# Triton-AI/Triton-Racer-Sim

Measured on AMD Instinct MI355X. Metric: env-steps/s (whole node) at N envs x 120x160 RGB, higher is better.
Workload: dtype f32 state / f64 nearest-point / u8 image; 1 GPU; 1024 envs/GPU x 1 GPU, bicycle physics + L1 nearest point + 120x160 RGB pinhole rasteriser = BASELINE configs[2], generated_track 1185 pts, synthetic controls seed 0x5EED, auto-reset; envs_total=1024, envs_per_gpu=1024, img_h=120, img_w=160, depth=False, steps_per_launch=1, step_mode=resident worker (posted steps), prewarm_steps=8400, launcher=self

## Files before the change

### triton-racer-sim_amd/csrc/trsim_env.hpp

```cpp
#pragma once
#include <hip/hip_runtime.h>

#include <algorithm>
#include <cstdint>
#include <cstring>
#include <string>

#include "../../include/trsim.h"
#include "trsim_device.hpp"
#include "trsim_mem.hpp"
#include "trsim_tables.hpp"

namespace trsim { struct Resident; struct Comm; }

struct trs_env {
    trs_config cfg{};
    int device = 0, n = 0, H = 0, W = 0, cu_count = 0;
    hipStream_t sP = nullptr;
    hipEvent_t ev[8] = {};
    trsim::DevBuf<> slab;
    trsim::DevBuf<uint8_t> img[2];
    bool uniform_ok[2] = {false, false};
    trsim::DevBuf<float> depth[2];
    trsim::DevBuf<> blob_p;
    trsim::DevBuf<> blob_r;
    trsim::DevBuf<float> tangent, start_yaw;
    trsim::DevBuf<float4> cam;
    trsim::DevBuf<float> cam_pitch;
    trsim::DevBuf<float> dpitch;
    bool hilly = false;
    trsim::HillBlock hill_host{};
    trs_camera camera{};
    bool lens_on = false;
    trsim::LensTables lens;
    trsim::DevBuf<> lens_dev;
    size_t lens_pal_off = 0;
    bool light_on = false;
    const float* light = nullptr;
    trsim::DevBuf<float> light_own;
    trsim::DevBuf<unsigned long long> stats;
    trsim::DevBuf<double> loc_q; trsim::DevBuf<int32_t> loc_out; int loc_cap = 0;
    trsim::DevBuf<uint8_t> pre;
    trs_pre_config frame_filter{}; bool has_frame_filter = false, filter_dynamic = false;
    trsim::PinnedBuf<> pinned;
    trsim::DevBuf<int32_t> mux_state; int mux_tick = 0;
    trsim::DevBuf<uint8_t> tmp_in, tmp_out; trsim::DevBuf<float> tmp_f; size_t tmp_cap = 0;
    trsim::DevBuf<int> hsv_tab;
    trsim::DevBuf<unsigned> dyn_tab;
    trsim::DevBuf<> edge_scratch;
    trsim::PParams pp{};
    trsim::RParams rp{};
    trsim::TrackTables tab;
    bool track_loaded = false;
    int lds_p = 0, lds_r = 0, pts_bytes = 0;
    uint64_t step_count = 0;
// ... 62 lines not shown
```

### triton-racer-sim_amd/csrc/trsim_hip.hip

```cpp
#include <hip/hip_runtime.h>

#include <algorithm>
#include <array>
#include <cmath>
#include <cstdint>
#include <cstdio>
#include <cstring>
#include <string>
#include <utility>
#include <vector>

#include "../../include/trsim.h"
#include "../../include/trsim_spec.h"
#include "trsim_device.hpp"
#include "trsim_env.hpp"
#include "trsim_internal.hpp"
#include "trsim_tables.hpp"


#define TRS_EXPORT extern "C" __attribute__((visibility("default")))

namespace {


// ... 204 lines not shown
            if (sidx < 0) cam = lcam_prev[j];
            else {
                while (__hip_atomic_load(&pprog[j], __ATOMIC_ACQUIRE, __HIP_MEMORY_SCOPE_WORKGROUP) < sidx + 1) __builtin_amdgcn_s_sleep(2);
                cam = lcam[sidx * sp.cam_stride + j];
            }
            raster_lens_frame(p, rth, lb, lcache, (unsigned)lds_off_hill, frame_desc<DEPTH>(p, img, dep, e), cam);
            continue;
        }
        if constexpr (DYN) {
            if ((e - e_begin) % kDynBatch != 0) continue;
            const int nbatch = (e_end - e_begin + kDynBatch - 1) / kDynBatch;
            const int it = (sidx - sp.r_first) * nbatch + (e - e_begin) / kDynBatch;
            float4 cams[kDynBatch];
#pragma unroll
            for (int bi = 0; bi < kDynBatch; ++bi) {
                const int eb = e + bi;
                cams[bi] = make_float4(0.f, 0.f, 0.f, 1.f);
                if (eb < e_end) {
                    const int j = eb - e_begin;
                    if (sidx < 0) cams[bi] = lcam_prev[j];
                    else {
                        while (__hip_atomic_load(&pprog[j], __ATOMIC_ACQUIRE, __HIP_MEMORY_SCOPE_WORKGROUP) < sidx + 1) __builtin_amdgcn_s_sleep(2);
                        cams[bi] = lcam[sidx * sp.cam_stride + j];
                    }
                }
            }
            (void)raster_dyn_batch<DEPTH, LIGHT>(p, sp.fp, rth, smem, cams, min(kDynBatch, e_end - e), img, dep, e, it, tid, lane, [](bool) { return false; },
                                                 LIGHT ? llight + (e - e_begin) * 8 : nullptr, lds_off_lpal);
            continue;
        }
        const FrameDesc fd = frame_desc<DEPTH>(p, img, dep, e);
        RasterThread rl = rth;
        if constexpr (LIGHT && !HILLS && !DYN) rl.pal_off = light_wave_palette(p, lds_off_lpal, llight + (e - e_begin) * 8, lfilt, wave, lane);
        if (!sp.skip_uniform) raster_uniform_rows<DEPTH>(p, rl, fd);
        float4 cam;
        const int j = e - e_begin;
        if (sidx < 0) {
            cam = lcam_prev[j];
        } else {
            while (__hip_atomic_load(&pprog[j], __ATOMIC_ACQUIRE, __HIP_MEMORY_SCOPE_WORKGROUP) < sidx + 1) __builtin_amdgcn_s_sleep(2);
            cam = lcam[sidx * sp.cam_stride + j];
        }
        raster_ground_rows<DEPTH>(p, rl, fd, cam);
    }
    }
    STAMP(5);
}

using StepKernel = void (*)(SParams);
template <Variant V> StepKernel step_kernel_of()
{
    if constexpr (variant_built(V)) return &trs_step_kernel<(V & kVDepth) != 0, (V & kVDyn) != 0, (V & kVHills) != 0, (V & kVLens) != 0, (V & kVLight) != 0>;
    else return nullptr;
}
template <Variant... V> std::array<StepKernel, kVariants> step_kernel_table(std::integer_sequence<Variant, V...>) { return {step_kernel_of<V>()...}; }
const std::array<StepKernel, kVariants> kStepKernels = step_kernel_table(std::make_integer_sequence<Variant, kVariants>{});

#undef STAMP_STATS
struct PreParams {
    const uint8_t* src; uint8_t* dst;
    const int* hsv_tab;
    int n_img, H, W, gpr, gpe, r0, r1;
    int dynamic, color, n_filters;
    float contrast, offset;
    double baseline;
    unsigned lo[4], hi[4];
    int dst_ch[4];
// ... 555 lines not shown
#define HIPCHK(call)                                                                              \
    do {                                                                                          \
        hipError_t _e = (call);                                                                   \
        if (_e != hipSuccess) return fail(TRS_ERR_DEVICE, std::string(#call) + ": " + hipGetErrorString(_e)); \
    } while (0)

inline size_t align_up(size_t v, size_t a) { return (v + a - 1) / a * a; }

}

namespace {

const uint8_t* latest_frame(const trs_env* e) { return e->cfg.render ? e->img[(e->step_count + 1) & 1].get() : nullptr; }
const float* latest_depth(const trs_env* e) { return (e->cfg.render && e->cfg.depth) ? e->depth[(e->step_count + 1) & 1].get() : nullptr; }

int grid_of(const trs_env* e) { return (e->n + e->pp.envs_per_wg - 1) / e->pp.envs_per_wg; }

trsim::LdsFit handle_fit(const trs_env* e, Variant v, int lds_step) { return trsim::lds_fit(lds_step, e->pp.envs_per_wg, e->H, e->W, v, trsim::resident_on(e)); }
int steps_that_fit(const trs_env* e, Variant v, int lds_step) { return trsim::steps_that_fit(lds_step, e->pp.envs_per_wg, e->H, e->W, v); }
Variant variant_now(const trs_env* e) { return trsim::variant_of(e) & (e->track_loaded ? ~0u : ~kVHills); }

int sync_all(trs_env* e)
{
    if (e->res) { int rc = trsim::resident_quiesce(e); if (rc) return rc; }
    HIPCHK(hipStreamSynchronize(e->sP));
    return trsim::check_fault(e);
}

int quiesce(trs_env* e) { return e->res ? trsim::resident_quiesce(e) : TRS_OK; }

bool resident_steps(const trs_env* e) { return trsim::resident_on(e); }

int launch_step(trs_env* e, const float* st, const float* th, const float* br, const uint8_t* rs, int synth,
                int n_phys, int r_first, int r_last, uint64_t step_base, bool keep_uniform = false)
{
    const Variant v = trsim::variant_of(e);
    const StepKernel kernel = kStepKernels[v];
    if (!kernel) return fail(TRS_ERR_STATE, "internal error: no step kernel is built for this combination of camera, track, frame filter and lighting");
    SParams sp;
    const bool dyn = (v & kVDyn) != 0;
    sp.ph = e->pp;
    sp.ph.ctl_steer = st; sp.ph.ctl_thr = th; sp.ph.ctl_brk = br; sp.ph.ctl_reset = rs; sp.ph.ctl_stride = e->seq_stride;
    sp.ph.synth = synth; sp.ph.n_steps = n_phys; sp.ph.write_cam = 1; sp.ph.step_off = (uint32_t)step_base;
    sp.ra = e->rp;
    sp.img0 = e->img[0].get(); sp.img1 = e->img[1].get();
    sp.dep0 = e->depth[0].get(); sp.dep1 = e->depth[1].get();
    sp.n_phys = n_phys; sp.r_first = r_first; sp.r_last = r_last;
    sp.step_base = (unsigned)step_base;
    sp.lds_off_phys = e->lds_off_phys;
    sp.cam_stride = e->pp.envs_per_wg;
    const StepLds lds = step_lds_layout(e->lds_step, sp.cam_stride, e->H, e->W, v, n_phys);
    sp.lds_off_cam = lds.cam; sp.lds_off_prog = lds.prog;
    sp.skip_uniform = 0;
    for (int r = r_first; r <= r_last; ++r) {
        const int b = (int)((step_base + (uint64_t)(int64_t)r) & 1u);
        if (keep_uniform && r_first == r_last && e->uniform_ok[b] && !dyn && !e->lens_on && !e->light_on) sp.skip_uniform = 1;
        else e->uniform_ok[b] = !dyn && !e->lens_on && !e->light_on;
    }
    sp.fp = trsim::fparams_of(e, lds.dyn);
    hipLaunchKernelGGL(kernel, dim3(grid_of(e)), dim3(kBlock), lds.total, e->sP, sp);
    HIPCHK(hipGetLastError());
    return TRS_OK;
}

int run_camera_steps(trs_env* e, const float* st, const float* th, const float* br, const uint8_t* rs, int synth, int n, int per_launch, bool keep_uniform = false)
{
    const uint64_t s0 = e->step_count;
    int rc = TRS_OK;
    if (n == 1) {
        rc = launch_step(e, st, th, br, rs, synth, 1, 0, 0, s0, keep_uniform);
    } else {
        const int kmax = std::max(1, std::min(per_launch, steps_that_fit(e, trsim::variant_of(e), e->lds_step)));
        for (int done = 0; done < n && !rc;) {
            const int k = std::min(kmax, n - done);
            const size_t co = (size_t)done * (size_t)e->seq_stride;
            rc = launch_step(e, st ? st + co : st, th ? th + co : th, br ? br + co : br, done == 0 ? rs : nullptr, synth, k, done == 0 ? 0 : -1, k - 2, s0 + done);
            done += k;
        }
        if (!rc) rc = launch_step(e, st, th, br, nullptr, synth, 0, -1, -1, s0 + n);
    }
    if (rc) return rc;
    e->step_count += (uint64_t)n;
    return TRS_OK;
}

int run_physics_steps(trs_env* e, const float* st, const float* th, const float* br, const uint8_t* rs, int synth, int n, int per_launch)
{
    for (int done = 0; done < n;) {
        const int now = std::min(per_launch, n - done);
        PParams p = e->pp;
        const size_t co = (size_t)done * (size_t)e->seq_stride;
        p.ctl_steer = st ? st + co : st; p.ctl_thr = th ? th + co : th; p.ctl_brk = br ? br + co : br; p.ctl_reset = done == 0 ? rs : nullptr;
        p.ctl_stride = e->seq_stride;
        p.synth = synth; p.n_steps = now; p.write_cam = 0; p.step_off = (uint32_t)e->step_count;
        hipLaunchKernelGGL(trs_physics_kernel, dim3((e->n + kPhysBlock / 64 - 1) / (kPhysBlock / 64)), dim3(kPhysBlock), e->lds_p, e->sP, p);
        HIPCHK(hipGetLastError());
        e->step_count += (uint64_t)now;
        done += now;
    }
    return TRS_OK;
}

}
// ... 28 lines not shown
{
    e->cfg = *cfg; e->device = device; e->n = cfg->n_envs; e->H = cfg->img_h; e->W = cfg->img_w;
    hipDeviceProp_t prop;
    HIPCHK(hipGetDeviceProperties(&prop, device));
    e->cu_count = prop.multiProcessorCount > 0 ? prop.multiProcessorCount : 256;
    HIPCHK(hipStreamCreateWithFlags(&e->sP, hipStreamNonBlocking));
    for (auto& ev : e->ev) HIPCHK(hipEventCreate(&ev));
    HIPCHK(hipEventCreateWithFlags(&e->ev_order, hipEventDisableTiming));

    const size_t n = (size_t)e->n, fa = align_up(n * 4, 256), ba = align_up(n, 256);
    const size_t slab_bytes = fa * (10 + 2 + 3) + ba * 3;
    HIPCHK(e->slab.alloc(slab_bytes));
    HIPCHK(hipMemsetAsync(e->slab.get(), 0, slab_bytes, e->sP));
    unsigned char* c = e->slab.get();
    auto takef = [&](float*& ptr) { ptr = reinterpret_cast<float*>(c); c += fa; };
    PParams& k = e->pp;
    takef(k.x); takef(k.y); takef(k.z); takef(k.yaw); takef(k.v); takef(k.speed); takef(k.cte);
    takef(k.ep_return); takef(k.last_return); takef(k.steer_filt);
    k.seg_idx = reinterpret_cast<int32_t*>(c); c += fa;
    k.ep_len = reinterpret_cast<int32_t*>(c); c += fa;
    takef(e->ctl_steer); takef(e->ctl_thr); takef(e->ctl_brk);
    k.done = c; c += ba; k.pending = c; c += ba; e->ctl_reset = c; c += ba;
    HIPCHK(e->stats.alloc(64 * sizeof(unsigned long long)));
    HIPCHK(hipMemsetAsync(e->stats.get(), 0, e->stats.bytes(), e->sP));
    HIPCHK(e->cam.alloc((size_t)kRing * n * sizeof(float4)));
    HIPCHK(hipMemsetAsync(e->cam.get(), 0, e->cam.bytes(), e->sP));
    HIPCHK(e->cam_pitch.alloc((size_t)kRing * n * sizeof(float)));
    HIPCHK(hipMemsetAsync(e->cam_pitch.get(), 0, e->cam_pitch.bytes(), e->sP));
    k.stats = e->stats.get(); k.cam = e->cam.get();
    RParams& r = e->rp;
    r.stats = e->stats.get();
    if (cfg->render) {
        e->img_bytes = n * (size_t)e->H * e->W * 3;
        for (int b = 0; b < 2; ++b) {
            HIPCHK(e->img[b].alloc(e->img_bytes));
            HIPCHK(hipMemsetAsync(e->img[b].get(), 0, e->img_bytes, e->sP));
            if (cfg->depth) {
                HIPCHK(e->depth[b].alloc(n * (size_t)e->H * e->W * 4));
                HIPCHK(hipMemsetAsync(e->depth[b].get(), 0, e->depth[b].bytes(), e->sP));
            }
        }
    }
    k.n_envs = e->n; k.env_id_base = cfg->env_id_base;
    k.envs_per_wg = (e->n + e->cu_count - 1) / e->cu_count;
    r.n_envs = e->n; r.envs_per_wg = k.envs_per_wg;
    r.H = e->H; r.W = e->W; r.gpr = e->W / 4; r.gpe = r.gpr * e->H; r.depth = (cfg->render && cfg->depth) ? 1 : 0;
    k.dt = cfg->dt; k.max_steer = cfg->max_steer; k.inv_wheelbase = cfg->inv_wheelbase; k.accel_max = cfg->accel_max;
    k.drag_lin = cfg->drag_lin; k.roll_res = cfg->roll_res; k.brake_max = cfg->brake_max; k.v_max = cfg->v_max;
    k.v_rev_max = cfg->v_rev_max; k.offtrack_cte = cfg->offtrack_cte; k.offtrack_penalty = cfg->offtrack_penalty;
    k.cam_fwd = cfg->cam_fwd; k.auto_reset = cfg->auto_reset; k.seed = cfg->seed;
    if (r.gpr > kBlock) return fail(TRS_ERR_LIMIT, "img_w too large: more 4-pixel groups per row than threads per workgroup");
    if (r.gpr > kRasterThreads) return fail(TRS_ERR_LIMIT, "img_w too large: more 4-pixel groups per row than raster threads");
    r.rows_per_pass = kRasterThreads / r.gpr;
    HIPCHK(e->fault.alloc(64, hipHostMallocMapped | hipHostMallocCoherent));
    *e->fault.get() = 0ull;
    k.fault = e->fault.get(); r.fault = e->fault.get();
    HIPCHK(hipStreamSynchronize(e->sP));
    return TRS_OK;
}


}

TRS_EXPORT int trs_create(const trs_config* cfg, int device, trs_env** out)
{
    if (!cfg || !out) return fail(TRS_ERR_ARG, "null argument");
// ... 534 lines not shown
    int o[3] = {t[0], t[1], t[2]};
    if (c.color_filter_enabled) {
        const int r = t[0], g = t[1], b = t[2];
        const int v = std::max(r, std::max(g, b)), vmin = std::min(r, std::min(g, b)), diff = v - vmin;
        const int sdiv = v ? (int)std::lrint((255 << 12) / (1.0 * v)) : 0;
        const int hdiv = diff ? (int)std::lrint((180 << 12) / (6.0 * diff)) : 0;
        const int sat = (diff * sdiv + (1 << 11)) >> 12;
        int h = (v == r) ? (g - b) : ((v == g) ? (b - r + 2 * diff) : (r - g + 4 * diff));
        h = (h * hdiv + (1 << 11)) >> 12;
        if (h < 0) h += 180;
        const int hh = std::min(h, 255), ss = std::min(sat, 255);
        for (int f = 0; f < c.n_filters; ++f) {
            const bool in = hh >= c.hsv_lo[f][0] && hh <= c.hsv_hi[f][0] && ss >= c.hsv_lo[f][1] && ss <= c.hsv_hi[f][1] &&
                            v >= c.hsv_lo[f][2] && v <= c.hsv_hi[f][2];
            o[c.dst_channel[f]] = in ? 255 : 0;
        }
    }
    return (uint32_t)o[0] | ((uint32_t)o[1] << 8) | ((uint32_t)o[2] << 16);
}

int leading_uniform_rows(const std::vector<uint32_t>& pal, int H)
{
    int u = 0;
    while (u < H && pal[4 * u] == pal[4 * u + 1] && pal[4 * u] == pal[4 * u + 2] && pal[4 * u] == pal[4 * u + 3]) ++u;
    return u;
}

int upload_palette(trs_env* e)
{
    if (!e->track_loaded || !e->cfg.render) return TRS_OK;
    std::vector<uint32_t> pal(e->tab.palette);
    if (e->has_frame_filter && !e->filter_dynamic && !e->light_on)
        for (auto& c : pal) c = filter_colour(e->frame_filter, c);
    e->rp.uni_rows = (e->hilly || e->lens_on) ? 0 : leading_uniform_rows(pal, e->H);
    e->uniform_ok[0] = e->uniform_ok[1] = false;
    { int rq = sync_all(e); if (rq) return rq; }
    HIPCHK(hipMemcpy(e->blob_r.get() + e->rp.off_pal, pal.data(), pal.size() * 4, hipMemcpyHostToDevice));
    if (e->lens_on && e->lens_dev.get()) {
        std::vector<uint32_t> lp(e->lens.palette);
        if (e->has_frame_filter && !e->filter_dynamic)
            for (auto& c : lp) c = filter_colour(e->frame_filter, c);
        HIPCHK(hipMemcpy(e->lens_dev.get() + e->lens_pal_off, lp.data(), lp.size() * 4, hipMemcpyHostToDevice));
    }
    if (e->hilly || e->light_on) {
        const bool flt = e->has_frame_filter && !e->filter_dynamic;
        trsim::HillBlock& hb = e->hill_host;
        std::vector<uint32_t> sky(e->tab.sky);
        hb.far_rgb = e->tab.far_rgb;
        hb.filt = flt ? 1 : 0;
        hb.light = e->light_on ? e->light : nullptr;
        if (flt) {
            const trs_pre_config& c = e->frame_filter;
            if (!e->light_on) {
                for (auto& v : sky) v = filter_colour(c, v);
                hb.far_rgb = filter_colour(c, hb.far_rgb);
            }
            { int rc = ensure_hsv_table(e); if (rc) return rc; }
            hb.f_color = c.color_filter_enabled; hb.f_nfilters = c.n_filters; hb.f_contrast = c.contrast_ratio; hb.f_offset = c.contrast_offset;
            for (int k = 0; k < 4; ++k) {
                hb.f_lo[k] = (unsigned)trsim::pack_hsv(c.hsv_lo[k]);
                hb.f_hi[k] = (unsigned)trsim::pack_hsv(c.hsv_hi[k]);
                hb.f_dst[k] = c.dst_channel[k];
            }
            hb.hsv_tab = e->hsv_tab.get();
        }
        if (e->hilly) HIPCHK(hipMemcpy(e->blob_r.get() + hb.off_sky, sky.data(), sky.size() * 4, hipMemcpyHostToDevice));
        HIPCHK(hipMemcpy(e->blob_r.get() + trsim::hill_block_offset(e->rp.blob_bytes), &hb, sizeof hb, hipMemcpyHostToDevice));
    }
    return TRS_OK;
// ... 533 lines not shown
    out[0] = e->d2h_bytes; out[1] = e->h2d_bytes; out[2] = e->step_count; out[3] = 0;
    return TRS_OK;
}

TRS_EXPORT const char* trs_last_error(void) { return g_err.c_str(); }

bool trs_internal_view(trs_env* e, TrsEnvView* v)
{
    if (!e || !v) return false;
    if (quiesce(e)) return false;
    v->device = e->device; v->n = e->n; v->H = e->H; v->W = e->W; v->render = e->cfg.render;
    v->stream = e->sP;
    v->latest_frame = e->step_count > 0 ? latest_frame(e) : nullptr;
    v->speed = e->pp.speed; v->seg_idx = e->pp.seg_idx; v->n_points = e->pp.np;
    v->ctl_steer = e->ctl_steer; v->ctl_thr = e->ctl_thr; v->ctl_brk = e->ctl_brk;
    v->step_count = e->step_count;
    v->stats = e->stats.get();
    return true;
}
void** trs_internal_pilot_slot(trs_env* e) { return e ? &e->pilot : nullptr; }
const trs_pilot_tuning* trs_internal_pilot_tuning(trs_env* e) { return e && e->has_pilot_tuning ? &e->pilot_tuning : nullptr; }
void trs_internal_set_pilot_tuning(trs_env* e, const trs_pilot_tuning* t)
{
    if (!e) return;
    e->has_pilot_tuning = t != nullptr;
    if (t) e->pilot_tuning = *t;
}
int trs_internal_fail(int code, const std::string& msg) { return fail(code, msg); }
void trs_internal_count(trs_env* e, uint64_t d2h, uint64_t h2d) { if (e) { e->d2h_bytes += d2h; e->h2d_bytes += h2d; } }
int trs_internal_step_launch(trs_env* e, const float* d_st, const float* d_th, const float* d_br)
{
    if (!e || !e->track_loaded) return fail(TRS_ERR_STATE, "no track loaded");
    { int rq = quiesce(e); if (rq) return rq; }
    const int rc = e->cfg.render ? run_camera_steps(e, d_st, d_th, d_br, nullptr, 0, 1, 1, true) : run_physics_steps(e, d_st, d_th, d_br, nullptr, 0, 1, 1);
    if (!rc) trsim::resident_note_launch(e);
    return rc;
}
int trs_internal_replay_launch(trs_env* e, const float* st, const float* th, const float* br, const uint8_t* rs, int synth, uint64_t step)
{
    if (e->cfg.render) return launch_step(e, st, th, br, rs, synth, 1, 0, 0, step);
    PParams p = e->pp;
    p.ctl_steer = st; p.ctl_thr = th; p.ctl_brk = br; p.ctl_reset = rs; p.ctl_stride = 0;
    p.synth = synth; p.n_steps = 1; p.write_cam = 0; p.step_off = (uint32_t)step;
    hipLaunchKernelGGL(trs_physics_kernel, dim3((e->n + kPhysBlock / 64 - 1) / (kPhysBlock / 64)), dim3(kPhysBlock), e->lds_p, e->sP, p);
    HIPCHK(hipGetLastError());
    return TRS_OK;
}
void trs_internal_note(const std::string& msg) { g_err = msg; }
int trsim::sync_handle(trs_env* e) { return sync_all(e); }
int trsim::quiesce_handle(trs_env* e) { return quiesce(e); }
int trsim::check_fault(trs_env* e)
{
    if (e->fault.get() && __atomic_load_n(e->fault.get(), __ATOMIC_ACQUIRE) != 0ull)
        return fail(TRS_ERR_DEVICE, "a step kernel found its dynamic LDS segment at a non-zero offset and refused to run: frames and state are stale");
    return TRS_OK;
}

#ifdef TRS_DEBUG_PROBES
__global__ __launch_bounds__(1024) void trs_debug_poison_kernel(unsigned pattern, int bytes, int spin)
{
    u4v* d = reinterpret_cast<u4v*>(smem);
    for (int i = threadIdx.x; i < bytes / 16; i += blockDim.x) d[i] = (u4v)(pattern);
    __syncthreads();
    const long long t0 = clock64();
    while (clock64() - t0 < spin) __builtin_amdgcn_s_sleep(8);
}

// ... 34 lines not shown
```

### triton-racer-sim_amd/csrc/trsim_plan.hpp

```cpp
#pragma once
#include <cstddef>
#include <string>
#include <vector>

#include "trsim_tables.hpp"

#ifndef TRS_RASTER_WAVES
#define TRS_RASTER_WAVES 8
#endif

namespace trsim {

constexpr int kRasterThreads = 64 * TRS_RASTER_WAVES;
constexpr int kPhysBlock = 256;
constexpr int kCamDepth = 4;
constexpr int kSlotWords = 20;
constexpr int kLensPalBytes = 513 * 16;
constexpr int kDynTabWords = 512 + 768 + 4 + 256;

using Variant = unsigned;
constexpr Variant kVDepth = 1, kVDyn = 2, kVHills = 4, kVLens = 8, kVLight = 16, kVariants = 32;
constexpr Variant variant_bits(bool depth, bool dyn, bool hills, bool lens, bool light)
{
    return (depth ? kVDepth : 0u) | (dyn ? kVDyn : 0u) | (hills ? kVHills : 0u) | (lens ? kVLens : 0u) | (light ? kVLight : 0u);
// ... 74 lines not shown
    return wlds_slot_off(epw) + (size_t)kCamDepth * epw * kSlotWords * 4 + (size_t)epw * 64;
}

struct WorkerLds { int ctl, dyn, hill, light, total; };
TRS_HD inline int worker_lds_light(int hill, int H, Variant v) { return (hill + tabs_lds_bytes(H, v) + 15) & ~15; }
TRS_HD inline WorkerLds worker_lds_layout(int lds_step, int epw, int H, int W, Variant v)
{
    WorkerLds L;
    L.ctl = (lds_step + 15) & ~15;
    int end = (int)(L.ctl + wlds_bytes(epw) + 16);
    L.dyn = (end + 15) & ~15;
    if (v & kVDyn) end = L.dyn + dyn_lds_bytes(H);
    L.hill = (end + 15) & ~15;
    if (v & (kVHills | kVLens)) end = L.hill + tabs_lds_bytes(H, v);
    L.light = worker_lds_light(L.hill, H, v);
    L.total = (v & kVLight) ? L.light + light_lds_extra(H, W, kCamDepth * epw, (v & kVHills) != 0, (v & kVDyn) != 0) : end;
    return L;
}

inline int steps_that_fit(int lds_step, int epw, int H, int W, Variant v)
{
    int n = 0;
    while (n < 16 && step_lds_layout(lds_step, epw, H, W, v, n + 1).total <= 160 * 1024) ++n;
    return n;
}
inline bool resident_fits(int lds_step, int epw, int H, int W, Variant v) { return worker_lds_layout(lds_step, epw, H, W, v).total <= 160 * 1024; }
enum class LdsFit { ok, no_launch, no_worker };
inline LdsFit lds_fit(int lds_step, int epw, int H, int W, Variant v, bool resident)
{
    if (steps_that_fit(lds_step, epw, H, W, v) < 1) return LdsFit::no_launch;
    return resident && !resident_fits(lds_step, epw, H, W, v) ? LdsFit::no_worker : LdsFit::ok;
}

struct TrackLayout {
    struct Phys { int off_py, off_pz, off_tan, tan_in_lds, off_gstart, off_gpts, blob_bytes, off_scratch, pts_bytes, lds_p; } p;
    struct Raster { int map_pitch_b, off_rowtab, off_pal, off_depth, off_sky, blob_bytes, lds_r; } r;
    int lds_off_phys, lds_step;
};
int track_layout(const TrackTables& T, int H, bool render, int envs_per_wg, TrackLayout& L, std::string& err);
void pack_track_images(const TrackTables& T, int H, const TrackLayout& L, std::vector<unsigned char>& phys, std::vector<unsigned char>& raster);

}
```

### triton-racer-sim_amd/csrc/trsim_resident.hip

```cpp
#include <hip/hip_runtime.h>

#include <algorithm>
#include <array>
#include <atomic>
#include <chrono>
#include <cstdint>
#include <cstdlib>
#include <cstddef>
#include <cstring>
#include <mutex>
#include <string>
#include <utility>

#include "../../include/trsim.h"
#include "../../include/trsim_spec.h"
#include "trsim_device.hpp"
#include "trsim_env.hpp"
#include "trsim_internal.hpp"

#define TRS_EXPORT extern "C" __attribute__((visibility("default")))

namespace trsim {

constexpr int kSlots = 8;
// ... 12 lines not shown

struct Mailbox {
    alignas(64) uint64_t close;
    uint64_t posted;
    alignas(64) uint64_t exited;
    uint64_t consumed;
    uint64_t error;
    uint64_t started;
    alignas(64) uint64_t done[kSlots];
    alignas(64) WEntry ring[kSlots];
};

struct DevCtl {
    alignas(64) unsigned long long word;
    alignas(64) WEntry ring[kSlots];
    alignas(64) unsigned arrive[kSlots][8][16];
    alignas(64) unsigned top[kSlots][16];
    alignas(64) unsigned checkin[16];
    alignas(64) unsigned decision[16];
};

struct WParams {
    PParams ph;
    RParams ra;
    uint8_t *img0, *img1;
    float *dep0, *dep1;
    Mailbox* mb;
    DevCtl* dc;
    unsigned long long start;
    unsigned long long idle_ticks, life_ticks, safety_ticks;
    unsigned long long checkin_ticks;
    int lds_off_phys, lds_off_ctl, n_blocks;
    int lds_off_hill;
    FParams fp;
};
#ifndef TRS_RESIDENT_DIAG
#define TRS_RESIDENT_DIAG 0
#endif
constexpr int kDiag = TRS_RESIDENT_DIAG;

constexpr unsigned kDefaultLifeUs = 50000;
#ifndef TRS_PHYS_PRIO_MAX_ENVS
#define TRS_PHYS_PRIO_MAX_ENVS 1
#endif
constexpr unsigned kRetryMs0 = 100;

struct Resident {
    bool enabled = false, running = false;
    bool broken = false;
    PinnedBuf<Mailbox> mb;
    DevBuf<DevCtl> dc;
    hipStream_t sC = nullptr;
    uint64_t base = 0;
    uint64_t seen_done = 0;
    bool launched = false;
    bool fell_back = false;
    bool dc_ready = false; uint64_t dc_ready_for = 0;
    std::chrono::steady_clock::time_point t_launch{};
    std::chrono::steady_clock::time_point t_fallback{};
    unsigned retry_ms = kRetryMs0;
    unsigned idle_us = 2000;
    unsigned life_us = kDefaultLifeUs;
    PinnedBuf<> hctl;
    size_t hctl_slot = 0;
    int lds_bytes = 0, lds_off_ctl = 0, lds_off_dyn = 0, lds_off_hill = 0;
    long long pw_capacity_envs = 0;
    int pw_capacity_lds = -1;
};

}

namespace {

using namespace trsim;
using u64 = unsigned long long;

constexpr u64 kExitBit = 1ull << 63, kAbortBit = 1ull << 62, kCountMask = kAbortBit - 1;
constexpr u64 kExitNormal = 1ull, kExitNotCoresident = 2ull;
constexpr u64 kCloseLeave = 1ull, kCloseCancel = 2ull;
constexpr int kFellBack = trsim::kResidentFellBack;

constexpr int kMaxDevices = 64;
struct DeviceSlot { std::recursive_mutex mu; trs_env* owner = nullptr; };
DeviceSlot g_dev[kMaxDevices];
struct DevLock {
    std::unique_lock<std::recursive_mutex> lk;
    explicit DevLock(const trs_env* e) : lk(g_dev[(unsigned)e->device % kMaxDevices].mu) {}
};
inline DeviceSlot& slot_of(const trs_env* e) { return g_dev[(unsigned)e->device % kMaxDevices]; }
// ... 384 lines not shown
        }
        if (D.forwarder) {
            u64 t0 = 0;
            for (unsigned spins = 0; D.fwd < s; ++spins) {
                forward_arrivals(wp, l, D.fwd, lane);
                if (lds_load64(l.word) & kAbortBit) break;
                __builtin_amdgcn_s_sleep(2);
                if ((spins & 1023u) == 1023u) {
                    const u64 now = (u64)wall_clock64();
                    if (t0 == 0) t0 = now;
                    else if (now - t0 > wp.safety_ticks) { worker_abort(wp, l, 4u); break; }
                }
            }
        }
        return;
    }

    const RasterThread rth = raster_thread(p, smem, tid);
    trsim::LensBlock lb{};
    LensCacheWorker<DEPTH> lcache;
    if constexpr (LENS) {
        lb = *reinterpret_cast<const trsim::LensBlock*>(p.blob + trsim::lens_block_offset(p.blob_bytes));
        lens_cache_load(p, rth, lb, lcache);
    }
    int nu = 0, ng = 0;
    for (int v = rth.vstart; v < p.uni_rows; v += p.rows_per_pass) ++nu;
    for (int v = rth.vground; v < p.H; v += p.rows_per_pass) ++ng;
#pragma unroll
    for (int off = 32; off >= 1; off >>= 1) { nu = max(nu, __shfl_xor(nu, off, 64)); ng = max(ng, __shfl_xor(ng, off, 64)); }
    nu *= DEPTH ? 2 : 1; ng *= DEPTH ? 2 : 1;
    int own = 0;
    for (int j = wave; j < n_loc; j += kRasterThreads / 64) ++own;
    const int nuni = nu * n_loc, nstep = (nu + ng) * n_loc + 2 * own;
    const int lag = (2 * nstep + nuni <= 63) ? 3 : 2;
    unsigned char* optr = nullptr;
    {
        unsigned char* const tab[14] = {(unsigned char*)P.x, (unsigned char*)P.y, (unsigned char*)P.z, (unsigned char*)P.yaw, (unsigned char*)P.v,
                                        (unsigned char*)P.speed, (unsigned char*)P.cte, (unsigned char*)P.seg_idx, (unsigned char*)P.ep_return,
                                        (unsigned char*)P.ep_len, (unsigned char*)P.steer_filt, (unsigned char*)P.last_return,
                                        (unsigned char*)P.done, (unsigned char*)P.pending};
#pragma unroll
        for (int k = 0; k < 14; ++k) optr = lane == k ? tab[k] : optr;
    }
    Duties none{false, false, 0};
    u64 owed = wp.start;
    const bool probe = (kDiag & 4) && blockIdx.x == 7 && wave == 0;
    auto now_clk = [&]() -> u64 { u64 t; asm volatile("s_memtime %0\n\ts_waitcnt lgkmcnt(0)" : "=s"(t) :: "memory"); return t; };
    u64 t_post = 0, t_pose = 0, t_vm = 0, t_all = 0, t_mark = probe ? now_clk() : 0;
    for (u64 s = wp.start;; ++s) {
        const int r = (int)(s - wp.start);
        if (owed < s && (lds_load64(l.word) & kCountMask) <= s) {
            drain_vmem();
            for (; owed < s; ++owed) raster_arrive(l, owed, lane);
        }
        const u64 tp0 = probe ? now_clk() : 0;
        if (!wait_posted(wp, l, none, s, lane)) {
            drain_vmem();
            for (; owed < s; ++owed) raster_arrive(l, owed, lane);
            if (probe && lane == 0) {
                t_all = now_clk() - t_mark;
                atomicAdd(&p.stats[40], t_post); atomicAdd(&p.stats[41], t_pose); atomicAdd(&p.stats[42], t_vm); atomicAdd(&p.stats[43], t_all);
                atomicAdd(&p.stats[44], (u64)r);
            }
            return;
        }
        if (probe) t_post += now_clk() - tp0;
        uint8_t* const img = (s & 1ull) ? wp.img1 : wp.img0;
// ... 90 lines not shown
                    else if (lane < 14) __hip_atomic_store((__attribute__((address_space(1))) unsigned char*)(uintptr_t)optr + e, (unsigned char)(lane == 12 ? tel : 0u), __ATOMIC_RELAXED, __HIP_MEMORY_SCOPE_SYSTEM);
                }
            }
            continue;
        }
        if constexpr (LIGHT && !HILLS && !DYN) {
            for (int j = 0; j < n_loc; ++j) {
                const FrameDesc fd = frame_desc<DEPTH>(p, img, dep, e_begin + j);
                if (!wait_lds_ge(wp, l, nullptr, &l.pprog[j], r + 1, 3u, lane)) return;
                const float* const sl = l.slot + ((size_t)(r & (kCamDepth - 1)) * epw + j) * kSlotWords;
                const float4 cam = *reinterpret_cast<const float4*>(sl);
                const bool mine = (j % (kRasterThreads / 64)) == wave;
                unsigned tel = 0;
                if (mine) tel = __float_as_uint(sl[4 + min(lane, 12)]);
                RasterThread rl = rth;
                rl.pal_off = light_wave_palette(p, lds_off_lpal, lring + ((size_t)(r & (kCamDepth - 1)) * epw + j) * 8, lfilt, wave, lane);
                asm volatile("s_waitcnt lgkmcnt(0)" :: "v"(cam.x), "v"(cam.y), "v"(cam.z), "v"(cam.w), "v"(tel) : "memory");
                if (lane == 0) __hip_atomic_fetch_add(&l.rread[j], 1, __ATOMIC_RELAXED, __HIP_MEMORY_SCOPE_WORKGROUP);
                raster_uniform_rows<DEPTH>(p, rl, fd);
                if (j == 0)
                    while (s - owed >= keep) {
                        wait_vmcnt_le((int)(s - owed - 1) * nstep + nu);
                        raster_arrive(l, owed++, lane);
                    }
                raster_ground_rows<DEPTH>(p, rl, fd, cam);
                if (mine && !(kDiag & 2)) {
                    const size_t e = (size_t)(e_begin + j);
                    if (lane < 12) __hip_atomic_store((__attribute__((address_space(1))) unsigned*)(uintptr_t)optr + e, tel, __ATOMIC_RELAXED, __HIP_MEMORY_SCOPE_SYSTEM);
                    else if (lane < 14) __hip_atomic_store((__attribute__((address_space(1))) unsigned char*)(uintptr_t)optr + e, (unsigned char)(lane == 12 ? tel : 0u), __ATOMIC_RELAXED, __HIP_MEMORY_SCOPE_SYSTEM);
                }
            }
            continue;
        }
        const bool sweep = ahead == 0;
        if (sweep)
            for (int j = 0; j < n_loc; ++j) raster_uniform_rows<DEPTH>(p, rth, frame_desc<DEPTH>(p, img, dep, e_begin + j));
        for (int j = 0; j < n_loc; ++j) {
            const FrameDesc fd = frame_desc<DEPTH>(p, img, dep, e_begin + j);
            if (!sweep) raster_uniform_rows<DEPTH>(p, rth, fd);
            if (j == 0)
                while (s - owed >= keep) {
                    const u64 tv0 = probe ? now_clk() : 0;
                    if (!(kDiag & 1)) wait_vmcnt_le((int)(s - owed - 1) * nstep + (sweep ? nuni : nu));
                    if (probe) t_vm += now_clk() - tv0;
                    raster_arrive(l, owed++, lane);
                }
            const u64 tq0 = probe ? now_clk() : 0;
            if (!wait_lds_ge(wp, l, nullptr, &l.pprog[j], r + 1, 3u, lane)) return;
            if (probe) t_pose += now_clk() - tq0;
            const float* const sl = l.slot + ((size_t)(r & (kCamDepth - 1)) * epw + j) * kSlotWords;
            const float4 cam = *reinterpret_cast<const float4*>(sl);
            const bool mine = (j % (kRasterThreads / 64)) == wave;
            unsigned tel = 0;
            if (mine) tel = __float_as_uint(sl[4 + min(lane, 12)]);
            asm volatile("s_waitcnt lgkmcnt(0)" :: "v"(cam.x), "v"(cam.y), "v"(cam.z), "v"(cam.w), "v"(tel) : "memory");
            if (lane == 0) __hip_atomic_fetch_add(&l.rread[j], 1, __ATOMIC_RELAXED, __HIP_MEMORY_SCOPE_WORKGROUP);
            if constexpr (LENS) raster_lens_frame(p, rth, lb, lcache, (unsigned)wp.lds_off_hill, fd, cam);
            else raster_ground_rows<DEPTH>(p, rth, fd, cam);
            if (mine && !(kDiag & 2)) {
                const size_t e = (size_t)(e_begin + j);
                if (lane < 12) __hip_atomic_store((__attribute__((address_space(1))) unsigned*)(uintptr_t)optr + e, tel, __ATOMIC_RELAXED, __HIP_MEMORY_SCOPE_SYSTEM);
                else if (lane < 14) __hip_atomic_store((__attribute__((address_space(1))) unsigned char*)(uintptr_t)optr + e, (unsigned char)(lane == 12 ? tel : 0u), __ATOMIC_RELAXED, __HIP_MEMORY_SCOPE_SYSTEM);
            }
        }
    }
}

using WorkerKernel = void (*)(WParams);
template <Variant V> WorkerKernel worker_kernel_of()
{
    if constexpr (variant_built(V)) return &trs_worker_kernel<(V & kVDepth) != 0, (V & kVDyn) != 0, (V & kVHills) != 0, (V & kVLens) != 0, (V & kVLight) != 0>;
    else return nullptr;
}
template <Variant... V> std::array<WorkerKernel, kVariants> worker_kernel_table(std::integer_sequence<Variant, V...>) { return {worker_kernel_of<V>()...}; }
const std::array<WorkerKernel, kVariants> kWorkerKernels = worker_kernel_table(std::make_integer_sequence<Variant, kVariants>{});

// ... 181 lines not shown
    }
    const WorkerLds L = worker_lds_layout(e->lds_step, e->pp.envs_per_wg, e->H, e->W, variant_of(e));
    R->lds_off_ctl = L.ctl; R->lds_off_dyn = L.dyn; R->lds_off_hill = L.hill; R->lds_bytes = L.total;
    if (R->lds_bytes > 160 * 1024)
        return trs_internal_fail(TRS_ERR_LIMIT, e->hilly ? "the resident worker's LDS state and the per-env row tables of a track with elevation do not fit beside this track's tables: use TRS_STEP_LAUNCH"
                                                : e->lens_on ? "the resident worker's LDS state and the lens camera's palette do not fit beside this track's tables: use TRS_STEP_LAUNCH"
                                                : e->light_on ? "the resident worker's LDS state and the lit palettes of scene lighting do not fit beside this track's tables: use TRS_STEP_LAUNCH"
                                                            : "too many envs per workgroup for the resident worker's LDS state");
    return TRS_OK;
}

int evict(trs_env* other);

int worker_launch(trs_env* e, uint64_t start)
{
    Resident* R = e->res;
    Mailbox* mb = R->mb.get();
    { int rc = worker_fits(e); if (rc) return rc; }
    const WorkerKernel kernel = e->cfg.render ? kWorkerKernels[variant_of(e)] : nullptr;
    if (e->cfg.render && !kernel)
        return trs_internal_fail(TRS_ERR_STATE, "internal error: no resident worker is built for this combination of camera, track, frame filter and lighting");
    {
        DeviceSlot& D = slot_of(e);
        trs_env* const other = D.owner;
        if (other && other != e && other->res && other->res->running) (void)evict(other);
        D.owner = e;
    }
    host_store(&mb->exited, 0); host_store(&mb->consumed, start); host_store(&mb->error, 0);
    host_store(&mb->close, 0); host_store(&mb->started, 0);
    WParams wp{};
    wp.ph = e->pp; wp.ph.synth = 0; wp.ph.write_cam = 0; wp.ph.n_steps = 0; wp.ph.step_off = 0; wp.ph.ctl_stride = 0;
    wp.ra = e->rp;
    wp.img0 = e->img[0].get(); wp.img1 = e->img[1].get(); wp.dep0 = e->depth[0].get(); wp.dep1 = e->depth[1].get();
    e->uniform_ok[0] = e->uniform_ok[1] = false;
    wp.mb = mb; wp.dc = R->dc.get();
    wp.start = start;
    wp.idle_ticks = (unsigned long long)R->idle_us * 100ull;
    wp.life_ticks = (unsigned long long)R->life_us * 100ull;
    wp.safety_ticks = 200000000ull;
    wp.checkin_ticks = 200000ull;
    wp.lds_off_phys = e->lds_off_phys; wp.lds_off_ctl = R->lds_off_ctl; wp.lds_off_hill = R->lds_off_hill;
    const int grid = e->cfg.render ? (e->n + e->pp.envs_per_wg - 1) / e->pp.envs_per_wg : (e->n + kPwEnvs - 1) / kPwEnvs;
    wp.n_blocks = grid;
    if (!(R->dc_ready && R->dc_ready_for == start)) hipLaunchKernelGGL(trs_worker_init_kernel, dim3(1), dim3(256), 0, e->sP, R->dc.get(), (u64)start);
    R->dc_ready = false;
    if (e->cfg.render) {
        wp.fp = fparams_of(e, R->lds_off_dyn);
        hipLaunchKernelGGL(kernel, dim3(grid), dim3(kBlock), R->lds_bytes, e->sP, wp);
    } else {
        hipLaunchKernelGGL(trs_physics_worker_kernel, dim3(grid), dim3(kPwBlock), R->lds_bytes, e->sP, wp);
    }
    RCHK(hipGetLastError());
    R->running = true;
    R->t_launch = std::chrono::steady_clock::now();
    return TRS_OK;
}

int worker_error(trs_env* e)
{
    const uint64_t err = host_load(&e->res->mb->error);
    if (!err) return TRS_OK;
    e->res->broken = true;
    static const char* const what[] = {"", "waiting for a post", "camera ring back-pressure", "waiting for the physics team", "forwarding the last arrivals",
                                       "team barrier of the dynamic-brightness batch", "", "abort injected by trs_resident_debug_abort (test hook)", "",
                                       "dynamic LDS segment not at offset 0"};
    const unsigned code = (unsigned)(err >> 32);
    return trs_internal_fail(TRS_ERR_DEVICE, std::string("resident worker gave up (") + (code < 10 ? what[code] : "?") + ") in workgroup " +
                                                 std::to_string((unsigned)err));
}

int fall_back_to_launches(trs_env* e, uint64_t consumed, const char* why)
{
    Resident* R = e->res;
    const uint64_t posted = host_load(&R->mb->posted);
    R->enabled = false;
    R->fell_back = true;
    R->t_fallback = std::chrono::steady_clock::now();
    if (consumed > R->seen_done) R->seen_done = consumed;
    for (uint64_t s = consumed; s < posted; ++s) {
        const WEntry& en = R->mb->ring[s & (kSlots - 1)];
        if (en.seq != s + 1 || en.seq_lo != s + 1)
            return trs_internal_fail(TRS_ERR_DEVICE, "resident worker: the post of step " + std::to_string(s) + " is no longer in the ring");
        int rc = trs_internal_replay_launch(e, en.steer, en.thr, en.brk, en.reset, (int)en.synth, s);
        if (rc) return rc;
    }
    R->launched = true;
    R->base = R->seen_done = e->step_count;
    for (int k = 0; k < kSlots; ++k) { host_store(&R->mb->ring[k].seq, 0); host_store(&R->mb->ring[k].seq_lo, 0); host_store(&R->mb->done[k], 0); }
    trs_internal_note(std::string("resident worker: ") + why + " - another process's worker holds CUs of this GPU; the handle has gone back to TRS_STEP_LAUNCH "
                      "(resident mode is tried again by itself after " + std::to_string(R->retry_ms) + " ms; trs_get_step_mode tells)");
    return kFellBack;
}

int handle_exit(trs_env* e, bool relaunch = true)
{
    Resident* R = e->res;
    RCHK(hipStreamSynchronize(e->sP));
    R->running = false;
    int rc = worker_error(e);
    if (rc) return rc;
    const uint64_t consumed = host_load(&R->mb->consumed), posted = host_load(&R->mb->posted);
    if (host_load(&R->mb->exited) == kExitNotCoresident)
        return fall_back_to_launches(e, consumed, "the launch did not get every CU within 2 ms");
    if (consumed > R->seen_done) R->seen_done = consumed;
    if (host_load(&R->mb->started)) R->retry_ms = kRetryMs0;
    if (consumed < posted && relaunch) return worker_launch(e, consumed);
    if (consumed == posted) {
        hipLaunchKernelGGL(trs_worker_init_kernel, dim3(1), dim3(256), 0, e->sP, R->dc.get(), (u64)consumed);
        if (hipGetLastError() == hipSuccess) { R->dc_ready = true; R->dc_ready_for = consumed; }
    }
    return TRS_OK;
}

int evict(trs_env* other)
{
    Resident* R = other->res;
    int rc = TRS_OK;
    if (R->running) {
        host_store(&R->mb->close, kCloseLeave);
        rc = handle_exit(other, false);
    }
    return rc < 0 ? rc : TRS_OK;
}

int give_up_on_launch(trs_env* e)
{
    Resident* R = e->res;
    host_store(&R->mb->close, kCloseCancel);
    RCHK(hipStreamSynchronize(e->sP));
    R->running = false;
    int rc = worker_error(e);
    if (rc) return rc;
    return fall_back_to_launches(e, host_load(&R->mb->consumed), "the launch had not started after 250 ms");
}

int wait_done(trs_env* e, uint64_t s)
{
    Resident* R = e->res;
    if (s < R->seen_done) return TRS_OK;
    Mailbox* mb = R->mb.get();
    const auto t0 = std::chrono::steady_clock::now();
    auto fell_back = [&]() -> int {
        RCHK(hipStreamSynchronize(e->sP));
        R->launched = false;
        R->base = R->seen_done = e->step_count;
        return TRS_OK;
    };
    for (unsigned spins = 0;; ++spins) {
        if (host_load(&mb->done[s & (kSlots - 1)]) >= s + 1) { R->seen_done = s + 1; return TRS_OK; }
        if ((spins & 63u) == 63u) {
            if (R->running && host_load(&mb->exited)) {
                int rc = handle_exit(e);
                if (rc == kFellBack) return fell_back();
                if (rc) return rc;
                if (s < R->seen_done) return TRS_OK;
            } else if (!R->running) {
                if (host_load(&mb->posted) > R->seen_done) { int rc = worker_launch(e, R->seen_done); if (rc) return rc; }
            } else if ((spins & 4095u) == 4095u && !host_load(&mb->started) &&
                       std::chrono::steady_clock::now() - R->t_launch > std::chrono::milliseconds(250)) {
                int rc = give_up_on_launch(e);
                if (rc == kFellBack) return fell_back();
                if (rc) return rc;
            }
            if (host_load(&mb->error)) { (void)handle_exit(e); return worker_error(e); }
            if (std::chrono::steady_clock::now() - t0 > std::chrono::seconds(10))
// ... 258 lines not shown
```

Measured before the change: 108.3 million env-steps/s.

## Skip redundant uniform-row rasterisation in resident worker after double-buffered frames are primed

```diff
diff --git a/triton-racer-sim_amd/csrc/trsim_env.hpp b/triton-racer-sim_amd/csrc/trsim_env.hpp
--- a/triton-racer-sim_amd/csrc/trsim_env.hpp
+++ b/triton-racer-sim_amd/csrc/trsim_env.hpp
@@ -20,7 +20,7 @@
     hipEvent_t ev[8] = {};
     trsim::DevBuf<> slab;
     trsim::DevBuf<uint8_t> img[2];
-    bool uniform_ok[2] = {false, false};
+    trsim::UniformRows uniform_ok;
     trsim::DevBuf<float> depth[2];
     trsim::DevBuf<> blob_p;
     trsim::DevBuf<> blob_r;
diff --git a/triton-racer-sim_amd/csrc/trsim_hip.hip b/triton-racer-sim_amd/csrc/trsim_hip.hip
--- a/triton-racer-sim_amd/csrc/trsim_hip.hip
+++ b/triton-racer-sim_amd/csrc/trsim_hip.hip
@@ -260,7 +260,7 @@
         const FrameDesc fd = frame_desc<DEPTH>(p, img, dep, e);
         RasterThread rl = rth;
         if constexpr (LIGHT && !HILLS && !DYN) rl.pal_off = light_wave_palette(p, lds_off_lpal, llight + (e - e_begin) * 8, lfilt, wave, lane);
-        if (!sp.skip_uniform) raster_uniform_rows<DEPTH>(p, rl, fd);
+        if (!((sp.skip_uniform >> (abs_step & 1u)) & 1)) raster_uniform_rows<DEPTH>(p, rl, fd);
         float4 cam;
         const int j = e - e_begin;
         if (sidx < 0) {
@@ -882,13 +882,12 @@
 bool resident_steps(const trs_env* e) { return trsim::resident_on(e); }
 
 int launch_step(trs_env* e, const float* st, const float* th, const float* br, const uint8_t* rs, int synth,
-                int n_phys, int r_first, int r_last, uint64_t step_base, bool keep_uniform = false)
+                int n_phys, int r_first, int r_last, uint64_t step_base)
 {
     const Variant v = trsim::variant_of(e);
     const StepKernel kernel = kStepKernels[v];
     if (!kernel) return fail(TRS_ERR_STATE, "internal error: no step kernel is built for this combination of camera, track, frame filter and lighting");
     SParams sp;
-    const bool dyn = (v & kVDyn) != 0;
     sp.ph = e->pp;
     sp.ph.ctl_steer = st; sp.ph.ctl_thr = th; sp.ph.ctl_brk = br; sp.ph.ctl_reset = rs; sp.ph.ctl_stride = e->seq_stride;
     sp.ph.synth = synth; sp.ph.n_steps = n_phys; sp.ph.write_cam = 1; sp.ph.step_off = (uint32_t)step_base;
@@ -901,24 +900,20 @@
     sp.cam_stride = e->pp.envs_per_wg;
     const StepLds lds = step_lds_layout(e->lds_step, sp.cam_stride, e->H, e->W, v, n_phys);
     sp.lds_off_cam = lds.cam; sp.lds_off_prog = lds.prog;
-    sp.skip_uniform = 0;
-    for (int r = r_first; r <= r_last; ++r) {
-        const int b = (int)((step_base + (uint64_t)(int64_t)r) & 1u);
-        if (keep_uniform && r_first == r_last && e->uniform_ok[b] && !dyn && !e->lens_on && !e->light_on) sp.skip_uniform = 1;
-        else e->uniform_ok[b] = !dyn && !e->lens_on && !e->light_on;
-    }
+    sp.skip_uniform = (int)e->uniform_ok.skip_mask(v);
+    if (r_first <= r_last) e->uniform_ok.rendered(v, step_base + (uint64_t)(int64_t)r_first, (uint64_t)(r_last - r_first + 1));
     sp.fp = trsim::fparams_of(e, lds.dyn);
     hipLaunchKernelGGL(kernel, dim3(grid_of(e)), dim3(kBlock), lds.total, e->sP, sp);
     HIPCHK(hipGetLastError());
     return TRS_OK;
 }
 
-int run_camera_steps(trs_env* e, const float* st, const float* th, const float* br, const uint8_t* rs, int synth, int n, int per_launch, bool keep_uniform = false)
+int run_camera_steps(trs_env* e, const float* st, const float* th, const float* br, const uint8_t* rs, int synth, int n, int per_launch)
 {
     const uint64_t s0 = e->step_count;
     int rc = TRS_OK;
     if (n == 1) {
-        rc = launch_step(e, st, th, br, rs, synth, 1, 0, 0, s0, keep_uniform);
+        rc = launch_step(e, st, th, br, rs, synth, 1, 0, 0, s0);
     } else {
         const int kmax = std::max(1, std::min(per_launch, steps_that_fit(e, trsim::variant_of(e), e->lds_step)));
         for (int done = 0; done < n && !rc;) {
@@ -1013,6 +1008,7 @@
     r.stats = e->stats.get();
     if (cfg->render) {
         e->img_bytes = n * (size_t)e->H * e->W * 3;
+        e->uniform_ok.invalidate();
         for (int b = 0; b < 2; ++b) {
             HIPCHK(e->img[b].alloc(e->img_bytes));
             HIPCHK(hipMemsetAsync(e->img[b].get(), 0, e->img_bytes, e->sP));
@@ -1613,9 +1609,9 @@
     std::vector<uint32_t> pal(e->tab.palette);
     if (e->has_frame_filter && !e->filter_dynamic && !e->light_on)
         for (auto& c : pal) c = filter_colour(e->frame_filter, c);
+    { int rq = sync_all(e); if (rq) return rq; }
     e->rp.uni_rows = (e->hilly || e->lens_on) ? 0 : leading_uniform_rows(pal, e->H);
-    e->uniform_ok[0] = e->uniform_ok[1] = false;
-    { int rq = sync_all(e); if (rq) return rq; }
+    e->uniform_ok.invalidate();
     HIPCHK(hipMemcpy(e->blob_r.get() + e->rp.off_pal, pal.data(), pal.size() * 4, hipMemcpyHostToDevice));
     if (e->lens_on && e->lens_dev.get()) {
         std::vector<uint32_t> lp(e->lens.palette);
@@ -2215,7 +2211,7 @@
 {
     if (!e || !e->track_loaded) return fail(TRS_ERR_STATE, "no track loaded");
     { int rq = quiesce(e); if (rq) return rq; }
-    const int rc = e->cfg.render ? run_camera_steps(e, d_st, d_th, d_br, nullptr, 0, 1, 1, true) : run_physics_steps(e, d_st, d_th, d_br, nullptr, 0, 1, 1);
+    const int rc = e->cfg.render ? run_camera_steps(e, d_st, d_th, d_br, nullptr, 0, 1, 1) : run_physics_steps(e, d_st, d_th, d_br, nullptr, 0, 1, 1);
     if (!rc) trsim::resident_note_launch(e);
     return rc;
 }
diff --git a/triton-racer-sim_amd/csrc/trsim_plan.hpp b/triton-racer-sim_amd/csrc/trsim_plan.hpp
--- a/triton-racer-sim_amd/csrc/trsim_plan.hpp
+++ b/triton-racer-sim_amd/csrc/trsim_plan.hpp
@@ -130,6 +130,27 @@
     return resident && !resident_fits(lds_step, epw, H, W, v) ? LdsFit::no_worker : LdsFit::ok;
 }
 
+constexpr bool variant_keeps_uniform(Variant v) { return !(v & (kVDyn | kVLens | kVLight)); }
+struct UniformRows {
+    bool ok[2] = {false, false};
+    void invalidate() { ok[0] = ok[1] = false; }
+    unsigned skip_mask(Variant v) const { return variant_keeps_uniform(v) ? (ok[0] ? 1u : 0u) | (ok[1] ? 2u : 0u) : 0u; }
+    void rendered(Variant v, unsigned long long first, unsigned long long n)
+    {
+        for (unsigned long long k = 0; k < n && k < 2; ++k) ok[(first + k) & 1ull] = variant_keeps_uniform(v);
+    }
+};
+
+TRS_HD inline bool worker_skips_uniform(unsigned mask, unsigned long long start, unsigned long long s) { return ((mask >> (s & 1ull)) & 1u) != 0 || s - start >= 2; }
+TRS_HD inline int worker_step_stores(int nstep, int nuni, bool skips) { return skips ? nstep - nuni : nstep; }
+TRS_HD inline int worker_wait_count(unsigned mask, unsigned long long start, unsigned long long owed, unsigned long long s, int nstep, int nuni, int uni_now)
+{
+    int n = uni_now;
+    for (unsigned long long q = owed + 1; q < s; ++q) n += worker_step_stores(nstep, nuni, worker_skips_uniform(mask, start, q));
+    return n;
+}
+TRS_HD inline int worker_lag(int nstep, int nuni, bool skipping) { return (2 * worker_step_stores(nstep, nuni, skipping) + (skipping ? 0 : nuni) <= 63) ? 3 : 2; }
+
 struct TrackLayout {
     struct Phys { int off_py, off_pz, off_tan, tan_in_lds, off_gstart, off_gpts, blob_bytes, off_scratch, pts_bytes, lds_p; } p;
     struct Raster { int map_pitch_b, off_rowtab, off_pal, off_depth, off_sky, blob_bytes, lds_r; } r;
diff --git a/triton-racer-sim_amd/csrc/trsim_resident.hip b/triton-racer-sim_amd/csrc/trsim_resident.hip
--- a/triton-racer-sim_amd/csrc/trsim_resident.hip
+++ b/triton-racer-sim_amd/csrc/trsim_resident.hip
@@ -68,6 +68,7 @@
     unsigned long long checkin_ticks;
     int lds_off_phys, lds_off_ctl, n_blocks;
     int lds_off_hill;
+    unsigned uni_mask;
     FParams fp;
 };
 #ifndef TRS_RESIDENT_DIAG
@@ -91,6 +92,7 @@
     uint64_t seen_done = 0;
     bool launched = false;
     bool fell_back = false;
+    uint64_t gen_start = 0; Variant gen_variant = 0;
     bool dc_ready = false; uint64_t dc_ready_for = 0;
     std::chrono::steady_clock::time_point t_launch{};
     std::chrono::steady_clock::time_point t_fallback{};
@@ -541,7 +543,8 @@
     int own = 0;
     for (int j = wave; j < n_loc; j += kRasterThreads / 64) ++own;
     const int nuni = nu * n_loc, nstep = (nu + ng) * n_loc + 2 * own;
-    const int lag = (2 * nstep + nuni <= 63) ? 3 : 2;
+    constexpr bool kSkipUniform = !DYN && !HILLS && !LIGHT && !LENS;
+    const int lag = worker_lag(nstep, nuni, kSkipUniform);
     unsigned char* optr = nullptr;
     {
         unsigned char* const tab[14] = {(unsigned char*)P.x, (unsigned char*)P.y, (unsigned char*)P.z, (unsigned char*)P.yaw, (unsigned char*)P.v,
@@ -698,16 +701,19 @@
             }
             continue;
         }
-        const bool sweep = ahead == 0;
+        const bool skipu = kSkipUniform && worker_skips_uniform(wp.uni_mask, wp.start, s);
+        const bool sweep = ahead == 0 && !skipu;
         if (sweep)
             for (int j = 0; j < n_loc; ++j) raster_uniform_rows<DEPTH>(p, rth, frame_desc<DEPTH>(p, img, dep, e_begin + j));
         for (int j = 0; j < n_loc; ++j) {
             const FrameDesc fd = frame_desc<DEPTH>(p, img, dep, e_begin + j);
-            if (!sweep) raster_uniform_rows<DEPTH>(p, rth, fd);
+            if (!sweep && !skipu) raster_uniform_rows<DEPTH>(p, rth, fd);
             if (j == 0)
                 while (s - owed >= keep) {
                     const u64 tv0 = probe ? now_clk() : 0;
-                    if (!(kDiag & 1)) wait_vmcnt_le((int)(s - owed - 1) * nstep + (sweep ? nuni : nu));
+                    if (!(kDiag & 1))
+                        wait_vmcnt_le(kSkipUniform ? worker_wait_count(wp.uni_mask, wp.start, owed, s, nstep, nuni, skipu ? 0 : (sweep ? nuni : nu))
+                                                   : (int)(s - owed - 1) * nstep + (sweep ? nuni : nu));
                     if (probe) t_vm += now_clk() - tv0;
                     raster_arrive(l, owed++, lane);
                 }
@@ -955,7 +961,8 @@
     wp.ph = e->pp; wp.ph.synth = 0; wp.ph.write_cam = 0; wp.ph.n_steps = 0; wp.ph.step_off = 0; wp.ph.ctl_stride = 0;
     wp.ra = e->rp;
     wp.img0 = e->img[0].get(); wp.img1 = e->img[1].get(); wp.dep0 = e->depth[0].get(); wp.dep1 = e->depth[1].get();
-    e->uniform_ok[0] = e->uniform_ok[1] = false;
+    wp.uni_mask = e->cfg.render ? e->uniform_ok.skip_mask(variant_of(e)) : 0u;
+    R->gen_start = start; R->gen_variant = e->cfg.render ? variant_of(e) : 0u;
     wp.mb = mb; wp.dc = R->dc.get();
     wp.start = start;
     wp.idle_ticks = (unsigned long long)R->idle_us * 100ull;
@@ -979,11 +986,19 @@
     return TRS_OK;
 }
 
+void worker_rendered(trs_env* e, uint64_t consumed)
+{
+    Resident* R = e->res;
+    if (e->cfg.render && consumed > R->gen_start) e->uniform_ok.rendered(R->gen_variant, R->gen_start, consumed - R->gen_start);
+    R->gen_start = std::max(R->gen_start, consumed);
+}
+
 int worker_error(trs_env* e)
 {
     const uint64_t err = host_load(&e->res->mb->error);
     if (!err) return TRS_OK;
     e->res->broken = true;
+    e->uniform_ok.invalidate();
     static const char* const what[] = {"", "waiting for a post", "camera ring back-pressure", "waiting for the physics team", "forwarding the last arrivals",
                                        "team barrier of the dynamic-brightness batch", "", "abort injected by trs_resident_debug_abort (test hook)", "",
                                        "dynamic LDS segment not at offset 0"};
@@ -1023,6 +1038,7 @@
     int rc = worker_error(e);
     if (rc) return rc;
     const uint64_t consumed = host_load(&R->mb->consumed), posted = host_load(&R->mb->posted);
+    worker_rendered(e, consumed);
     if (host_load(&R->mb->exited) == kExitNotCoresident)
         return fall_back_to_launches(e, consumed, "the launch did not get every CU within 2 ms");
     if (consumed > R->seen_done) R->seen_done = consumed;
@@ -1054,6 +1070,7 @@
     R->running = false;
     int rc = worker_error(e);
     if (rc) return rc;
+    worker_rendered(e, host_load(&R->mb->consumed));
     return fall_back_to_launches(e, host_load(&R->mb->consumed), "the launch had not started after 250 ms");
 }
 
```

Result: faster. 125.5 million env-steps/s, median of 6 (+15.9%).
